# facebookresearch/lightplane

Hardware: AMD Instinct MI355X
Metric: Mrays/sec fwd+bwd, 64^3x16ch triplane @128 samples; peak bwd mem (MB) (higher is better)
Workload: dtype f32

## Files before the change

lightplane_amd/csrc/lp_mfma_common.h:

```cpp
#pragma once
#include <stdlib.h>

#include "lp_device.h"
#include "lp_splat_walk.h"
#include "lp_host.h"
#include "lp_plane_range.h"

namespace lp {

typedef float f32x16 __attribute__((ext_vector_type(16)));

LP_DEV constexpr int featq(int q, int h) { return (q & 3) + 8 * (q >> 2) + 4 * h; }

#define LP_MFMA(a, b, c) __builtin_amdgcn_mfma_f32_32x32x2f32((a), (b), (c), 0, 0, 0)

LP_DEV int opaque_zero() {
  int z = 0;
  asm volatile("" : "+s"(z));
  return z;
}

constexpr int HID = 32;
constexpr int W_LD = 33;
constexpr int WAVES = 4;
// ... 5 lines not shown
constexpr int GM_VOXEL = 2;

struct MfmaParams {
  int64_t w_t1, w_t2, b_t1, b_t2;
  int64_t w_o1, w_o2, b_o1, b_o2;
  int64_t w_c1, w_c2, b_c1, b_c2;
  int ldc2;
  int hid, t2, oh, ch;
  int t1, tg, hin;
  int seg_blocks;
  int seg_fwd;
  uint32_t* relu_dump;
  int tm_rpw;
};

struct Lds {
  static constexpr int WT1 = 0;
  static constexpr int WT2 = WT1 + 32 * W_LD;
  static constexpr int WO1 = WT2 + 32 * W_LD;
  static constexpr int WC1 = WO1 + 32 * W_LD;
  static constexpr int BIAS = WC1 + 32 * W_LD;
  static constexpr int WO2 = BIAS + 4 * 32;
  static constexpr int WC2 = WO2 + 32;
  static constexpr int HB = WC2 + 32 * 4;
  static constexpr int INF = HB + 8;
  static constexpr int FWD_END = INF + MAX_INF;
};

LP_DEV f32x16 load_bias(const float* lds, int which, int h, int zo) {
  const float4* b = reinterpret_cast<const float4*>(lds + Lds::BIAS + which * 32 + 4 * h + zo);
  f32x16 acc;
#pragma unroll
  for (int j = 0; j < 4; ++j) {
    const float4 v = b[2 * j];
    acc[4 * j + 0] = v.x; acc[4 * j + 1] = v.y; acc[4 * j + 2] = v.z; acc[4 * j + 3] = v.w;
  }
  return acc;
}

LP_DEV int wave_min_i(int v) {
#pragma unroll
  for (int m = 32; m >= 1; m >>= 1) { const int o = __shfl_xor(v, m); v = o < v ? o : v; }
  return __builtin_amdgcn_readfirstlane(v);
}
struct WaveRanges {
  unsigned lo3, hi3;
  static constexpr unsigned G = 0x20080200u;
  LP_DEV unsigned mask(int s) const {
    s = __builtin_amdgcn_readfirstlane(s);
    const unsigned sss = (unsigned)(s < 511 ? s : 511) * 0x00100401u;
    return ((sss | G) - lo3) & ((hi3 | G) - sss) & G;
  }
  static constexpr unsigned bit(int g) { return 0x200u << (10 * g); }
};
constexpr int RANGE_MAX_S = 511;
LP_DEV WaveRanges wave_ranges_full() { return WaveRanges{0u, 0x1ff7fdffu}; }
template <int GM>
LP_DEV WaveRanges wave_plane_ranges(const LpRendererArgs& a, const Ray& ray, bool valid, bool plain) {
  WaveRanges w = wave_ranges_full();
  if (GM == GM_GENERIC) return w;
  const int S = a.march.num_samples;
  if (!plain || S > RANGE_MAX_S || __ballot(!valid) != 0) return w;
  const LpGrid* g = a.grid.grids;
  const int W = g[0].W, H = g[0].H, D = (GM == GM_TRIPLANE) ? g[1].D : g[0].D;
  const AxisSpans ax = ray_axis_spans(ray.ox, ray.oy, ray.oz, ray.dx, ray.dy, ray.dz, ray.near_t, ray.far_t, S, W, H, D);
#pragma unroll
  for (int p = 0; p < (GM == GM_TRIPLANE ? 3 : 1); ++p) {
    const SampleSpan sp = (GM == GM_TRIPLANE) ? plane_span(ax, p, S) : voxel_span(ax, S);
    const int lo = wave_min_i(sp.lo), hi = -wave_min_i(-sp.hi);
    if (p == 0) w.lo3 = w.hi3 = 0u;
    w.lo3 |= (unsigned)(hi < lo ? 511 : lo) << (10 * p);
    w.hi3 |= (unsigned)(hi < lo ? 0 : hi) << (10 * p);
  }
  if (GM == GM_VOXEL) {
    w.lo3 *= 0x00100401u;
    w.hi3 *= 0x00100401u;
  }
  w.lo3 = (unsigned)__builtin_amdgcn_readfirstlane((int)w.lo3);
  w.hi3 = (unsigned)__builtin_amdgcn_readfirstlane((int)w.hi3);
  return w;
}

template <int C>
LP_DEV void gather_tap(const float* data, int row, float w, int h, float (&x0)[C / 2]) {
  const float4* src = reinterpret_cast<const float4*>(data + (int64_t)(row < 0 ? 0 : row) * C + 4 * h);
#pragma unroll
  for (int j = 0; j < C / 8; ++j) {
    const float4 v = src[2 * j];
    x0[4 * j + 0] = fmaf(w, v.x, x0[4 * j + 0]);
    x0[4 * j + 1] = fmaf(w, v.y, x0[4 * j + 1]);
    x0[4 * j + 2] = fmaf(w, v.z, x0[4 * j + 2]);
    x0[4 * j + 3] = fmaf(w, v.w, x0[4 * j + 3]);
  }
}

template <int C>
LP_DEV void gather_taps4(const float* data, const int* row, const float* w, float keep, int h, float (&x0)[C / 2]) {
  float4 v[4][C / 8];
#pragma unroll
  for (int k = 0; k < 4; ++k) {
    const float4* src = reinterpret_cast<const float4*>(data + (int64_t)(row[k] < 0 ? 0 : row[k]) * C + 4 * h);
#pragma unroll
    for (int j = 0; j < C / 8; ++j) v[k][j] = src[2 * j];
  }
  __builtin_amdgcn_sched_barrier(0);
#pragma unroll
  for (int k = 0; k < 4; ++k) {
    const float wk = w[k] * keep;
#pragma unroll
    for (int j = 0; j < C / 8; ++j) {
      x0[4 * j + 0] = fmaf(wk, v[k][j].x, x0[4 * j + 0]);
      x0[4 * j + 1] = fmaf(wk, v[k][j].y, x0[4 * j + 1]);
      x0[4 * j + 2] = fmaf(wk, v[k][j].z, x0[4 * j + 2]);
      x0[4 * j + 3] = fmaf(wk, v[k][j].w, x0[4 * j + 3]);
    }
  }
}

template <int C, bool FENCED>
LP_DEV void gather_list(const LpGridList& gl, bool mask_oob, const Ray& ray, float x, float y, float z, int h,
                        float (&x0)[C / 2]) {
#pragma unroll
  for (int q = 0; q < C / 2; ++q) x0[q] = 0.0f;
  const float keep = (mask_oob && !point_in_bounds(x, y, z)) ? 0.0f : 1.0f;
  for (int g = 0; g < gl.n_grids; ++g) {
// ... 486 lines not shown
```

lightplane_amd/csrc/lp_plane_range.h:

```cpp
#pragma once
#include <math.h>

#if defined(__HIPCC__)
#define LP_HD __host__ __device__ inline
#else
#define LP_HD inline
#endif

namespace lp {

struct SampleSpan {
  int lo, hi;
};

LP_HD SampleSpan span_full(int S) { return SampleSpan{0, S - 1}; }
LP_HD SampleSpan span_none(int S) { return SampleSpan{S, -1}; }
LP_HD SampleSpan span_meet(SampleSpan a, SampleSpan b, int S) {
  const SampleSpan m{a.lo > b.lo ? a.lo : b.lo, a.hi < b.hi ? a.hi : b.hi};
  return m.lo > m.hi ? span_none(S) : m;
}
LP_HD SampleSpan span_hull(SampleSpan a, SampleSpan b) {
  return SampleSpan{a.lo < b.lo ? a.lo : b.lo, a.hi > b.hi ? a.hi : b.hi};
}

LP_HD SampleSpan axis_sample_span(float o, float d, float near_t, float far_t, int S, int size) {
  if (S < 2) return span_full(S);
  const float L = 1.0f + 1.0f / (float)size;
  const float per = (float)(S - 1) / (far_t - near_t);
  const float inv = 1.0f / d;
  float s0 = ((-L - o) * inv - near_t) * per;
  float s1 = ((L - o) * inv - near_t) * per;
  if (s0 > s1) { const float t = s0; s0 = s1; s1 = t; }
  const float err = 1.9073486e-6f * fabsf(per) * ((L + fabsf(o)) * fabsf(inv) + fabsf(near_t) + fabsf(far_t));
  if (!(err < 0.5f)) return span_full(S);
  if (!(s0 <= (float)S && s1 >= -1.0f)) return span_none(S);
  const int lo = (int)floorf(fmaxf(s0, 0.0f)) - 1;
  const int hi = (int)ceilf(fminf(s1, (float)(S - 1))) + 1;
  return SampleSpan{lo < 0 ? 0 : lo, hi > S - 1 ? S - 1 : hi};
}

struct AxisSpans {
  SampleSpan x, y, z;
};
LP_HD AxisSpans ray_axis_spans(float ox, float oy, float oz, float dx, float dy, float dz, float near_t, float far_t, int S, int W,
                               int H, int D) {
  return AxisSpans{axis_sample_span(ox, dx, near_t, far_t, S, W), axis_sample_span(oy, dy, near_t, far_t, S, H),
                   axis_sample_span(oz, dz, near_t, far_t, S, D)};
}
LP_HD SampleSpan plane_span(const AxisSpans& a, int g, int S) {
  return g == 0 ? span_meet(a.x, a.y, S) : (g == 1 ? span_meet(a.x, a.z, S) : span_meet(a.y, a.z, S));
}
LP_HD SampleSpan voxel_span(const AxisSpans& a, int S) { return span_meet(span_meet(a.x, a.y, S), a.z, S); }

}
```

lightplane_amd/csrc/lp_renderer_mfma.hip:

```cpp
#include "lp_mfma_common.h"
#include "lp_bf3.h"

namespace lp {

template <int C, int GM, int OCC, int NC, bool SEGF = false>
__global__ void __launch_bounds__(256, OCC) renderer_fwd_bf3(const LpRendererArgs a, const MfmaParams mp) {
  extern __shared__ __attribute__((aligned(16))) float lds[];
  stage_weights_bf3<C>(a, mp, lds, false, 256);
  __syncthreads();
  const float* sm = lds - Lds::BIAS;
  const char* fimg = reinterpret_cast<const char*>(lds) + LdsBf3<C>::FWD_IMG;
  const int lane = threadIdx.x & 63, wave = threadIdx.x >> 6;
  const int h = lane >> 5, r = lane & 31;
  const int seg_len = LP_SEG_LEN * mp.seg_blocks;
  const int n_seg = SEGF ? (a.march.num_samples + seg_len - 1) / seg_len : 1;
  const int blk = SEGF ? (int)blockIdx.x / n_seg : (int)blockIdx.x;
  const int seg = SEGF ? (int)blockIdx.x - blk * n_seg : 0;
  const int64_t ray_id = ((int64_t)blk * WAVES + wave) * RAYS_PER_WAVE + r;
  const bool valid = ray_id < a.rays.n_rays;
  const int64_t rid = valid ? ray_id : 0;
  const Ray ray = load_ray(a.rays, rid);
  float cb[16];
  {
    float enc[16];
    load_encoding(a, rid, h, enc);
    color_prebias_bf3<C>(sm, fimg, lane, enc, cb);
  }
  const int s_tot = a.march.num_samples + a.march.num_samples_inf;
  const int n_ckpt = ckpt_count(a.march);
  const float delta0 = (a.march.num_samples > 1) ? (ray.far_t - ray.near_t) / (float)(a.march.num_samples - 1) : 1.0f;
  float nlt = 0.0f, nlt_lo = 0.0f, t_prev = 1.0f, len = 0.0f, depth_prev = 0.0f;
  int s_last = s_tot - 1;
  float facc[4] = {0.0f, 0.0f, 0.0f, 0.0f};
  Sample<C> nx;
  Act<C> t;
  const int s_lo = SEGF ? seg * seg_len : 0;
  const int s_hi = SEGF ? ((s_lo + seg_len < s_tot) ? s_lo + seg_len : s_tot) : s_tot;
  const bool plain_march = !SEGF && a.march.num_samples_inf == 0 && !a.march.contract_coords && !a.scaffold && !(a.noise_sigma > 0.0f);
  const WaveRanges rg = wave_plane_ranges<GM>(a, ray, valid, plain_march);
  if (SEGF && s_lo > 0) {
    sample_geometry<C>(a, sm, ray, s_lo - 1, nx);
    depth_prev = nx.depth;
  }
  for (int s = s_lo; s < s_hi; ++s) {
    fetch_sample<C, GM, true>(a, sm, ray, s, h, nx, rg.mask(s));
    const float depth = nx.depth, occ = nx.occ;
#pragma unroll
    for (int q = 0; q < C / 2; ++q) t.x0[q] = nx.x0[q];
    const int zo = opaque_zero();
    const Heads hd = decode_bf3<C, NC>(sm, fimg, lane, cb, t, zo);
    const float delta = (s == 0) ? delta0 : depth - depth_prev;
    depth_prev = depth;
    float raw = hd.raw_o;
    if (a.noise_sigma > 0.0f) raw = raw + sample_noise(rid, s, a.rays.n_rays, s_tot, a.noise_seed) * a.noise_sigma;
    const float opacity = a.gain * softplus_f(raw) * occ;
    nlt_add(nlt, nlt_lo, opacity * delta);
    if (!SEGF && a.neg_log_t_ckpt && valid && h == 0) {
      const int ck = ckpt_index(s, a.march);
      if (ck >= 0) *reinterpret_cast<float2*>(a.neg_log_t_ckpt + (ray_id * n_ckpt + ck) * 2) = make_float2(nlt, nlt_lo);
    }
    const float tr = __expf(-nlt);
    const float w = t_prev - tr;
    t_prev = tr;
    len = fmaf(w, depth, len);
#pragma unroll
    for (int c = 0; c < NC; ++c) facc[c] = fmaf(w, sigmoid_f(hd.raw_c[c]) * occ, facc[c]);
    if (a.seg_prefix && valid && h == 0 && (((s + 1) % LP_SEG_LEN) == 0 || s == a.march.num_samples - 1)) {
      float4* dst = reinterpret_cast<float4*>(a.seg_prefix + (ray_id * segment_count(a.march) + s / LP_SEG_LEN) * 8);
      dst[0] = make_float4(len, facc[0], facc[1], facc[2]);
      dst[1] = make_float4(NC == 4 ? facc[3] : 0.0f, nlt, nlt_lo, 0.0f);
    }
    if (a.stop_neg_log_t > 0.0f && __ballot(valid && nlt < a.stop_neg_log_t) == 0) {
      s_last = s;
      break;
    }
  }
  if (!SEGF && valid && h == 0) {
    write_ray_outputs(a, ray_id, len, nlt, facc);
    if (a.neg_log_t_ckpt)
      *reinterpret_cast<float2*>(a.neg_log_t_ckpt + (ray_id * n_ckpt + n_ckpt - 1) * 2) = make_float2((float)s_last, nlt_lo);
  }
}

__global__ void __launch_bounds__(256) renderer_fwd_combine(const LpRendererArgs a, int seg_blocks) {
  const int64_t ray_id = (int64_t)blockIdx.x * 256 + threadIdx.x;
  if (ray_id >= a.rays.n_rays) return;
  const int S = a.march.num_samples;
  const int n_rec = segment_count(a.march), n_ckpt = ckpt_count(a.march);
  float4* rec = reinterpret_cast<float4*>(a.seg_prefix + ray_id * n_rec * 8);
  float n0 = 0.0f, n0_lo = 0.0f, l0 = 0.0f, f0[4] = {0.0f, 0.0f, 0.0f, 0.0f}, t0 = 1.0f;
  float nlt = 0.0f, nlt_lo = 0.0f, len = 0.0f, f[4] = {0.0f, 0.0f, 0.0f, 0.0f};
  for (int b = 0; b < n_rec; ++b) {
    if (b > 0 && b % seg_blocks == 0) {
      n0 = nlt; n0_lo = nlt_lo; l0 = len; t0 = __expf(-nlt);
      for (int c = 0; c < 4; ++c) f0[c] = f[c];
    }
    const float4 r0 = rec[2 * b], r1 = rec[2 * b + 1];
    nlt = n0; nlt_lo = n0_lo;
    nlt_add(nlt, nlt_lo, r1.y);
    nlt_add(nlt, nlt_lo, r1.z);
    len = fmaf(t0, r0.x, l0);
    f[0] = fmaf(t0, r0.y, f0[0]);
    f[1] = fmaf(t0, r0.z, f0[1]);
// ... 188 lines not shown
  return GM_GENERIC;
}

template <typename K>
static int set_lds(K kernel, size_t bytes) {
  const hipError_t e = hipFuncSetAttribute((const void*)kernel, hipFuncAttributeMaxDynamicSharedMemorySize, (int)bytes);
  if (e != hipSuccess) return set_error((int)e, "hipFuncSetAttribute: %s", hipGetErrorString(e));
  return LP_OK;
}

static unsigned n_blocks(const LpRendererArgs& a) {
  return (unsigned)((a.rays.n_rays + WAVES * RAYS_PER_WAVE - 1) / (WAVES * RAYS_PER_WAVE));
}

template <int C, int GM>
static int launch_fwd(const LpRendererArgs& a, const MfmaParams& mp, hipStream_t stream) {
  int rc;
  const bool nc3 = a.color_chn <= 3;
  if (renderer_tm_eligible(a)) {
    MfmaParams mt = mp;
    mt.tm_rpw = renderer_tm_rays_per_wave(a, 768);
    const size_t lds3 = (size_t)LdsBf3<C>::FWD_END;
    const unsigned nb = (unsigned)((a.rays.n_rays + WAVES * mt.tm_rpw - 1) / (WAVES * mt.tm_rpw));
    if (nc3) {
      if ((rc = set_lds(renderer_fwd_bf3_tm<C, GM, 3>, lds3))) return rc;
      hipLaunchKernelGGL((renderer_fwd_bf3_tm<C, GM, 3>), dim3(nb), dim3(256), lds3, stream, a, mt);
    } else {
      if ((rc = set_lds(renderer_fwd_bf3_tm<C, GM, 4>, lds3))) return rc;
      hipLaunchKernelGGL((renderer_fwd_bf3_tm<C, GM, 4>), dim3(nb), dim3(256), lds3, stream, a, mt);
    }
    return LP_OK;
  }
  static const int bf3_occ = getenv("LP_BF3_OCC") ? atoi(getenv("LP_BF3_OCC")) : 0;
  {
    const size_t lds3 = (size_t)LdsBf3<C>::FWD_END;
    const int occ = bf3_occ ? bf3_occ : (a.rays.n_rays > 2 * 32768 ? 3 : 2);
    static const bool seg_fwd = getenv("LP_SEG_FWD") == nullptr || atoi(getenv("LP_SEG_FWD")) != 0;
    if (a.seg_prefix && seg_fwd && !a.seg_forward_off) {
      MfmaParams ms = mp;
      const int n_rec = (a.march.num_samples + LP_SEG_LEN - 1) / LP_SEG_LEN;
      const int m = seg_blocks_for(n_blocks(a), n_rec, 512u);
      ms.seg_blocks = m;
      const unsigned nb = n_blocks(a) * (unsigned)((n_rec + m - 1) / m);
      if (nc3) {
        if ((rc = set_lds(renderer_fwd_bf3<C, GM, 2, 3, true>, lds3))) return rc;
        hipLaunchKernelGGL((renderer_fwd_bf3<C, GM, 2, 3, true>), dim3(nb), dim3(256), lds3, stream, a, ms);
      } else {
        if ((rc = set_lds(renderer_fwd_bf3<C, GM, 2, 4, true>, lds3))) return rc;
        hipLaunchKernelGGL((renderer_fwd_bf3<C, GM, 2, 4, true>), dim3(nb), dim3(256), lds3, stream, a, ms);
      }
      hipLaunchKernelGGL(renderer_fwd_combine, dim3((unsigned)((a.rays.n_rays + 255) / 256)), dim3(256), 0, stream, a, m);
      return LP_OK;
    }
#define LP_BF3_LAUNCH(OCCV, NCV)                                                                                  \
    do {                                                                                                          \
      if ((rc = set_lds(renderer_fwd_bf3<C, GM, OCCV, NCV>, lds3))) return rc;                                   \
      hipLaunchKernelGGL((renderer_fwd_bf3<C, GM, OCCV, NCV>), dim3(n_blocks(a)), dim3(256), lds3, stream, a, mp); \
    } while (0)
    if (occ >= 3) { if (nc3) LP_BF3_LAUNCH(3, 3); else LP_BF3_LAUNCH(3, 4); }
    else { if (nc3) LP_BF3_LAUNCH(2, 3); else LP_BF3_LAUNCH(2, 4); }
#undef LP_BF3_LAUNCH
    return LP_OK;
  }
}

#define LP_DISPATCH_GM(CALL, CV)                                   \
  switch (gm) {                                                    \
    case GM_TRIPLANE: rc = CALL(CV, GM_TRIPLANE); break;           \
    case GM_VOXEL: rc = CALL(CV, GM_VOXEL); break;                 \
    default: rc = CALL(CV, GM_GENERIC); break;                     \
  }

int renderer_forward_mfma(const LpRendererArgs& a, hipStream_t stream) {
  const MfmaParams mp = make_params(a);
  if (n_blocks(a) == 0) return LP_OK;
  const int gm = grid_mode(a);
  int rc;
#define LP_FWD(CV, GMV) launch_fwd<CV, GMV>(a, mp, stream)
  if (a.grid.channels == 16) { LP_DISPATCH_GM(LP_FWD, 16) } else { LP_DISPATCH_GM(LP_FWD, 32) }
#undef LP_FWD
  if (rc) return rc;
  return check_launch("renderer_fwd_mfma");
}

int renderer_backward_mfma(const LpRendererArgs& a, hipStream_t stream) {
  const MfmaParams mp = make_params(a);
  if (n_blocks(a) == 0) return LP_OK;
  return renderer_backward_mfma2(a, mp, grid_mode(a), stream);
}

}
```

lightplane_amd/csrc/lp_renderer_mfma_bwd.h:

```cpp
#pragma once
#include "lp_mfma_common.h"
#include <type_traits>

#include "lp_bf3.h"

namespace lp {

#ifdef LP_ASM_MARKS
#define LP_MARK(n) asm volatile("; LPMARK " n)
#else
#define LP_MARK(n)
#endif
typedef float f32x4 __attribute__((ext_vector_type(4)));
#define LP_MFMA16(a, b, c) __builtin_amdgcn_mfma_f32_16x16x4f32((a), (b), (c), 0, 0, 0)

constexpr int T_LD = 36;

LP_DEV constexpr int pi16(int m) { return m < 4 ? 2 * m : (m < 12 ? 2 * (m - 4) + 1 : 2 * (m - 8)); }

LP_DEV void lds_barrier() { asm volatile("s_waitcnt lgkmcnt(0)\n\ts_barrier" ::: "memory"); }

LP_DEV void tile_store_fm(float* tile, int r, int h, const float (&v)[16]) {
#pragma unroll
  for (int q = 0; q < 16; ++q) tile[featq(q, h) * T_LD + r] = v[q];
// ... 14 lines not shown
    acc = LP_MFMA16(a0.w, b0.w, acc);
    acc = LP_MFMA16(a1.x, b1.x, acc);
    acc = LP_MFMA16(a1.y, b1.y, acc);
    acc = LP_MFMA16(a1.z, b1.z, acc);
    acc = LP_MFMA16(a1.w, b1.w, acc);
    s += ((b0.x + b0.y) + (b0.z + b0.w)) + ((b1.x + b1.y) + (b1.z + b1.w));
  }
  db += s;
  return acc;
}

typedef __bf16 bf16x8_dw __attribute__((ext_vector_type(8)));
#define LP_MFMA16B(a, b, c) \
  __builtin_amdgcn_mfma_f32_16x16x32_bf16(__builtin_bit_cast(bf16x8_dw, (a)), __builtin_bit_cast(bf16x8_dw, (b)), (c), 0, 0, 0)
constexpr int LT_LIMB = rm_bytes(32);

LP_DEV u32x4_t limb_tile_operand(const char* p) {
  typedef __attribute__((address_space(3))) s16x4_t* lds_ptr;
  const s16x4_t a = __builtin_amdgcn_ds_read_tr16_b64_v4i16((lds_ptr)(p));
  const s16x4_t b = __builtin_amdgcn_ds_read_tr16_b64_v4i16((lds_ptr)(p + (rm_off(4, 0) - rm_off(0, 0))));
  const u32x2_t ua = __builtin_bit_cast(u32x2_t, a), ub = __builtin_bit_cast(u32x2_t, b);
  return (u32x4_t){ua.x, ua.y, ub.x, ub.y};
}
template <int STRIDE_BYTES>
LP_DEV f32x4 dw_quadrant_bf(const char* wave0b, int x_off, int y_off, int v0, int v1, f32x4 acc, f32x4& acc_db, unsigned onehot, bool do_db = true) {
  const u32x4_t oh = {onehot, onehot, onehot, onehot};
#pragma unroll 1
  for (int v = v0; v < v1; ++v) {
    const char* base = wave0b + v * STRIDE_BYTES;
    const u32x4_t b2 = limb_tile_operand(base + y_off + LT_LIMB);
    const u32x4_t a1 = limb_tile_operand(base + x_off);
    if (do_db) acc_db = LP_MFMA16B(oh, b2, acc_db);
    acc = LP_MFMA16B(a1, b2, acc);
    const u32x4_t b1 = limb_tile_operand(base + y_off);
    if (do_db) acc_db = LP_MFMA16B(oh, b1, acc_db);
    acc = LP_MFMA16B(a1, b1, acc);
    const u32x4_t a2 = limb_tile_operand(base + x_off + LT_LIMB);
    acc = LP_MFMA16B(a2, b1, acc);
  }
  return acc;
}

struct LdsB3 {
  static constexpr int XT = 0;
  static constexpr int YT = 32 * T_LD;
  static constexpr int TS = 2 * 32 * T_LD;
  static constexpr int PER_WAVE = TS + 5 * 32;
};
template <int C, int NW>
struct Bf3Lds {
  static constexpr int IMG_END = (NW == 8) ? LdsBf3<C>::BWD_END : LdsBf3Rm<C>::END;
  static constexpr int CB = IMG_END + NW * LdsB3::PER_WAVE * 4;
  static constexpr bool CB_LDS = (NW == 8) ? (C == 16) : (CB + NW * 64 * 16 * 4) * 2 <= 160 * 1024;
  static constexpr int TOTAL = CB + (CB_LDS ? NW * 64 * 16 * 4 : 0);
};

template <int C, int GM, bool PLAIN, int NC, int NW, bool SEG = false, bool DUMP = false, bool F32 = false>
__global__ void __launch_bounds__(64 * NW, NW == 8 ? 1 : 2) renderer_bwd_bf3(const LpRendererArgs a, const MfmaParams mp) {
  constexpr int DXL = F32 ? 3 : 2;
  constexpr bool DWB = !F32;
  using M = Lds;
  using L = LdsBf3<C>;
  using R = LdsBf3Rm<C>;
  using B = LdsB3;
  constexpr int WAVES3 = NW;
  extern __shared__ __attribute__((aligned(16))) float lds[];
  if (NW == 8) stage_weights_bf3<C>(a, mp, lds, true, 64 * NW);
  else stage_weights_rm<C>(a, mp, lds, 64 * NW);
  const float* const sm = lds - M::BIAS;
  const char* const fimg = reinterpret_cast<const char*>(lds) + L::FWD_IMG;
  const char* const bimg = reinterpret_cast<const char*>(lds) + L::BWD_IMG;
  const char* const rimg = reinterpret_cast<const char*>(lds);
  const int lane = threadIdx.x & 63;
  const int wave = __builtin_amdgcn_readfirstlane((int)(threadIdx.x >> 6));
  const int h = lane >> 5, r = lane & 31;
  float* const wave0 = reinterpret_cast<float*>(reinterpret_cast<char*>(lds) + Bf3Lds<C, NW>::IMG_END);
  float* const wv = wave0 + wave * B::PER_WAVE;
  float* const xt = wv + B::XT;
  float* const yt = wv + B::YT;
  float* const ts = wv + B::TS;

  constexpr bool seg_on = SEG;
  const int n_rec = seg_on ? segment_count(a.march) : 1;
  const int seg_len = LP_SEG_LEN * mp.seg_blocks;
  const int n_seg = seg_on ? (a.march.num_samples + seg_len - 1) / seg_len : 1;
  const int blk = seg_on ? (int)blockIdx.x / n_seg : (int)blockIdx.x;
  const int seg = seg_on ? (int)blockIdx.x - blk * n_seg : 0;
  const int64_t ray_id = ((int64_t)blk * WAVES3 + wave) * RAYS_PER_WAVE + r;
  const bool valid = ray_id < a.rays.n_rays;
  const int64_t rid = valid ? ray_id : 0;
  const Ray ray = load_ray(a.rays, rid);
  const int s_tot = a.march.num_samples + a.march.num_samples_inf;
  const int n_ckpt = ckpt_count(a.march);
  int s_last_w = s_tot - 1;
  float nlt_lo = 0.0f;
  if (a.neg_log_t_ckpt) {
    const float2 e2 = *reinterpret_cast<const float2*>(a.neg_log_t_ckpt + (rid * n_ckpt + n_ckpt - 1) * 2);
    s_last_w = __builtin_amdgcn_readfirstlane((int)e2.x);
    s_last_w = s_last_w < 0 ? 0 : (s_last_w > s_tot - 1 ? s_tot - 1 : s_last_w);
    nlt_lo = e2.y;
  }
  int s_begin = s_tot - 1;
  if (PLAIN) {
    __syncthreads();
  } else {
    if (lane == 0) ts[0] = (float)s_last_w;
    __syncthreads();
// ... 24 lines not shown
  }
  float dsum[16];
#pragma unroll
  for (int q = 0; q < 16; ++q) dsum[q] = 0.0f;
  float gfeat[4];
#pragma unroll
  for (int c = 0; c < 4; ++c)
    gfeat[c] = (valid && a.grad_feature && c < a.color_chn) ? a.grad_feature[rid * a.color_chn + c] : 0.0f;
  const float g_len = (valid && a.grad_ray_length) ? a.grad_ray_length[rid] : 0.0f;
  const float g_nlt = epilogue_grad_nlt(a, rid, valid, a.neg_log_t[rid],
                                        (valid && a.grad_neg_log_t) ? a.grad_neg_log_t[rid] : 0.0f, gfeat, 4);
  const bool want_params = a.grad_mlp_params != nullptr;
  const float delta0 = (a.march.num_samples > 1) ? (ray.far_t - ray.near_t) / (float)(a.march.num_samples - 1) : 1.0f;

  const int mi = (wave & 3) >> 1, ni = wave & 1;
  const int v0 = 4 * (wave >> 2);
  const int m16 = lane & 15, ka = lane >> 4;
  const int a_off = B::XT + (16 * mi + pi16(m16)) * T_LD + 8 * ka;
  const int b_off = B::YT + (16 * ni + pi16(m16)) * T_LD + 8 * ka;
  auto rho = [](int k) { return (k & 0x15) | ((k & 2) << 2) | ((k & 8) >> 2); };
  char* const xrow = reinterpret_cast<char*>(wv) + B::XT * 4 + rm_off(rho(r), 4 * h);
  char* const yrow = xrow + (B::YT - B::XT) * 4;
  const int xq_off = B::XT * 4 + rm_off(rho(8 * ka + (m16 >> 2)), 4 * (m16 & 3)) + 32 * mi;
  const int yq_off = B::YT * 4 + rm_off(rho(8 * ka + (m16 >> 2)), 4 * (m16 & 3)) + 32 * ni;
  f32x4 dq_b = {0, 0, 0, 0};
  auto onehot = [&](int li) -> unsigned { return (lane & 15) == li ? 0x3F803F80u : 0u; };
  const int a_off_t1 = (C == 16) ? B::XT + pi16(m16) * T_LD + 8 * ka : a_off;
  const int t1_v0 = (C == 16) ? 2 * (wave >> 1) : v0, t1_v1 = (C == 16) ? 2 * (wave >> 1) + 2 : v0 + 4;
  f32x4 dq_t1 = {0, 0, 0, 0}, dq_t2 = {0, 0, 0, 0}, dq_o1 = {0, 0, 0, 0}, dq_c1 = {0, 0, 0, 0};
  float db_t1 = 0.0f, db_t2 = 0.0f, db_o1 = 0.0f, db_c1 = 0.0f;
  float dwo2 = 0.0f, dwc2[4] = {0.0f, 0.0f, 0.0f, 0.0f};
  float dbo2 = 0.0f, dbc2[4] = {0.0f, 0.0f, 0.0f, 0.0f};
  const bool gg = a.grad_grid_list[0] != nullptr;

  float nlt = a.neg_log_t[rid];
  float suffix = 0.0f, p_next = 0.0f;
  if (seg_on) {
    const float4* pj = reinterpret_cast<const float4*>(a.seg_prefix + (rid * n_rec + s_begin / LP_SEG_LEN) * 8);
    const float4* pt = reinterpret_cast<const float4*>(a.seg_prefix + (rid * n_rec + n_rec - 1) * 8);
    const float4 j0 = pj[0], j1 = pj[1], t0 = pt[0];
    nlt = j1.y;
    nlt_lo = j1.z;
    if (seg < n_seg - 1) {
      float rest = g_len * (t0.x - j0.x);
      rest = fmaf(gfeat[0], t0.y - j0.y, rest);
      rest = fmaf(gfeat[1], t0.z - j0.z, rest);
      rest = fmaf(gfeat[2], t0.w - j0.w, rest);
      if (NC == 4) rest = fmaf(gfeat[3], pt[1].x - j1.x, rest);
      suffix = -rest;
    }
  }
  const WaveRanges rg = wave_plane_ranges<GM>(a, ray, valid, PLAIN && !SEG);
  Sample<C> nx;
  fetch_sample<C, GM, false, PLAIN>(a, sm, ray, s_begin, h, nx);
  for (int s = s_begin; s >= s_lo; --s) {
    const bool on = PLAIN || s <= s_last_w;
    const unsigned pm = rg.mask(s);
    const bool ggs = gg && pm != 0u;
    const float depth = nx.depth, occ = nx.occ, x = nx.x, y = nx.y, z = nx.z;
    float x0[C / 2];
#pragma unroll
    for (int q = 0; q < C / 2; ++q) x0[q] = nx.x0[q];
    const int zo = opaque_zero();
    const float* ldz = sm + zo;
    auto Af = [&](auto layer) {
      constexpr int l = decltype(layer)::value;
      if constexpr (NW == 8) return ASlots{fimg + zo, l == 0 ? L::CH_T1 : l == 1 ? L::CH_T2 : l == 2 ? L::CH_O1 : L::CH_C1};
      else return AColsFwd{rimg + zo + (l == 0 ? R::L_T1 : l == 1 ? R::L_T2 : l == 2 ? R::L_O1 : R::L_C1), l == 0 ? R::ST_T1 : R::ST_32};
    };
    auto Ab = [&](auto layer) {
      constexpr int l = decltype(layer)::value;
      if constexpr (NW == 8) return ASlots{bimg + zo, l == 0 ? L::CB_T1 : l == 1 ? L::CB_T2 : l == 2 ? L::CB_O1 : L::CB_C1};
      else return ARowsBwd{rimg + zo + (l == 0 ? R::L_T1 : l == 1 ? R::L_T2 : l == 2 ? R::L_O1 : R::L_C1), l == 0 ? R::ST_T1 : R::ST_32,
                           l == 0 ? C - 1 : 31};
    };
    using I0 = std::integral_constant<int, 0>; using I1 = std::integral_constant<int, 1>;
    using I2 = std::integral_constant<int, 2>; using I3 = std::integral_constant<int, 3>;

    LP_MARK("fwd");
    float h1[16];
    float e[16];
    unsigned ho_mask = 0, hc_mask = 0;
    Heads hd;
    {
      f32x16 acc;
      {
        acc = layer_bf3v<C / 16>(Af(I0{}), lane, x0, load_bias(sm, 0, h, zo));
#pragma unroll
        for (int q = 0; q < 16; ++q) h1[q] = relu_f(acc[q]);
      }
      acc = layer_bf3v<2>(Af(I1{}), lane, h1, load_bias(sm, 1, h, zo));
#pragma unroll
      for (int q = 0; q < 16; ++q) {
        e[q] = relu_f(acc[q]);
      }
      float ho[16], hc[16];
      {
        f32x16 acc_o = load_bias(sm, 2, h, zo), acc_c;
        if (CBL) {
#pragma unroll
          for (int i = 0; i < 4; ++i) {
            const float4 v = *reinterpret_cast<const float4*>(cbt + zo + ((i + cb_rot) & 3) * 4);
            acc_c[4 * i] = v.x; acc_c[4 * i + 1] = v.y; acc_c[4 * i + 2] = v.z; acc_c[4 * i + 3] = v.w;
          }
        } else {
#pragma unroll
          for (int q = 0; q < 16; ++q) acc_c[q] = cb[q];
        }
        layer2_bf3v<2>(Af(I2{}), Af(I3{}), lane, e, acc_o, acc_c);
#pragma unroll
        for (int q = 0; q < 16; ++q) {
          ho[q] = relu_f(acc_o[q]);
          hc[q] = relu_f(acc_c[q]);
        }
      }
      hd = heads_forward<NC>(sm, h, ho, hc, zo);
#pragma unroll
      for (int q = 0; q < 16; ++q) {
        ho_mask = mask_bit(ho_mask, ho[q], q);
        hc_mask = mask_bit(hc_mask, hc[q], q);
      }
      if constexpr (DUMP) {
        unsigned m1 = 0, m2 = 0, mo = 0, mc = 0;
#pragma unroll
        for (int q = 0; q < 16; ++q) {
          const unsigned bit = 1u << featq(q, h);
          m1 |= (h1[q] > 0.0f) ? bit : 0u;
          m2 |= (e[q] > 0.0f) ? bit : 0u;
          mo |= ((ho_mask >> q) & 1u) ? bit : 0u;
          mc |= ((hc_mask >> q) & 1u) ? bit : 0u;
        }
        m1 |= __shfl_xor(m1, 32); m2 |= __shfl_xor(m2, 32); mo |= __shfl_xor(mo, 32); mc |= __shfl_xor(mc, 32);
        if (valid && h == 0) {
          uint32_t* d = mp.relu_dump + (rid * s_tot + s) * 5;
          d[0] = m1; d[1] = m2; d[2] = mo; d[3] = mc; d[4] = on ? 1u : 2u;
        }
      }
      LP_SCHED_FENCE();
      if (want_params) {
        tile_store_fm(xt, r, h, ho);
        tile_store_fm(yt, r, h, hc);
      }
      LP_SCHED_FENCE();
    }

    LP_MARK("compositing");
    const float depth_prev =
        PLAIN ? ray.near_t + lin01((s > 0) ? s - 1 : 0, a.march.num_samples) * (ray.far_t - ray.near_t)
              : sample_depth_tab((s > 0) ? s - 1 : 0, a.march, ray.near_t, ray.far_t, sm + M::INF);
    const float delta = (s == 0) ? delta0 : depth - depth_prev;
    float raw = hd.raw_o;
    if (!PLAIN && a.noise_sigma > 0.0f)
      raw = raw + sample_noise(rid, s, a.rays.n_rays, s_tot, a.noise_seed) * a.noise_sigma;
    const float opacity = a.gain * softplus_f(raw) * occ;
    if (on && a.neg_log_t_ckpt) {
      const int ck = PLAIN ? ((((s + 1) % LP_NLT_CKPT) == 0 || s == s_tot - 1) ? s / LP_NLT_CKPT : -1)
                           : ckpt_index(s, a.march);
      if (ck >= 0) {
        const float2 c2 = *reinterpret_cast<const float2*>(a.neg_log_t_ckpt + (rid * n_ckpt + ck) * 2);
        nlt = c2.x;
        nlt_lo = c2.y;
      }
    }
    const float t_i = __expf(-nlt);
    nlt_add(nlt, nlt_lo, on ? -(opacity * delta) : 0.0f);
    if (!(nlt > 0.0f)) { nlt = 0.0f; nlt_lo = 0.0f; }
    const float t_im1 = __expf(-nlt);
    const float w = t_im1 - t_i;
    float sg[4];
    float p_i = g_len * depth;
#pragma unroll
    for (int c = 0; c < 4; ++c) {
      sg[c] = (c < NC) ? sigmoid_f(hd.raw_c[c]) : 0.0f;
      if (c < NC) p_i = fmaf(gfeat[c], sg[c] * occ, p_i);
    }
    suffix = on ? fmaf(t_i, p_i - p_next, suffix) : suffix;
    p_next = on ? p_i : p_next;
    const float d_a = suffix + g_nlt;
    const bool contrib = valid && on;
    const float dro = contrib ? d_a * delta * a.gain * occ * d_softplus_f(raw) : 0.0f;
    float drc[4];
#pragma unroll
    for (int c = 0; c < 4; ++c) drc[c] = (c < NC && contrib) ? w * gfeat[c] * occ * sg[c] * (1.0f - sg[c]) : 0.0f;

    LP_MARK("heads_bwd");
    float dhc[16];
    {
      const float* wc2 = sm + M::WC2 + 16 * h + opaque_zero();
#pragma unroll
      for (int j = 0; j < 4; ++j) {
#pragma unroll
        for (int i = 0; i < 4; ++i) {
          const int q = 4 * j + i;
          const float4 wc = *reinterpret_cast<const float4*>(wc2 + (8 * j + i) * 4);
          float v = drc[0] * wc.x;
          v = fmaf(drc[1], wc.y, v);
          v = fmaf(drc[2], wc.z, v);
          if (NC > 3) v = fmaf(drc[3], wc.w, v);
          dhc[q] = mask_apply(hc_mask, q, v);
        }
        LP_SCHED_FENCE();
      }
    }
    if (h == 0) {
      dbo2 += dro;
#pragma unroll
      for (int c = 0; c < NC; ++c) dbc2[c] += drc[c];
    }
    if (want_params) {
      if (h == 0) {
        ts[r] = dro;
#pragma unroll
        for (int c = 0; c < NC; ++c) ts[(1 + c) * 32 + r] = drc[c];
      }
      const float* xf = xt + r * T_LD + 16 * h;
      const float* yf = yt + r * T_LD + 16 * h;
      const float* tf = ts + 16 * h;
#pragma unroll
      for (int i = 0; i < 4; ++i) {
        const float4 hov = *reinterpret_cast<const float4*>(xf + 4 * i);
        const float4 hcv = *reinterpret_cast<const float4*>(yf + 4 * i);
        const float4 d0 = *reinterpret_cast<const float4*>(tf + 4 * i);
        dwo2 = fmaf(hov.x, d0.x, dwo2); dwo2 = fmaf(hov.y, d0.y, dwo2);
        dwo2 = fmaf(hov.z, d0.z, dwo2); dwo2 = fmaf(hov.w, d0.w, dwo2);
#pragma unroll
        for (int c = 0; c < NC; ++c) {
          const float4 dc = *reinterpret_cast<const float4*>(tf + (1 + c) * 32 + 4 * i);
          dwc2[c] = fmaf(hcv.x, dc.x, dwc2[c]); dwc2[c] = fmaf(hcv.y, dc.y, dwc2[c]);
          dwc2[c] = fmaf(hcv.z, dc.z, dwc2[c]); dwc2[c] = fmaf(hcv.w, dc.w, dwc2[c]);
        }
        LP_SCHED_FENCE();
      }
    }
    LP_SCHED_FENCE();

    LP_MARK("c1");
// ... 57 lines not shown
        if (want_params) limb_tile_store<2>(xrow, h1);
        acc = layer_dxv<2, DXL>(Ab(I1{}), lane, de, (f32x16){0}, want_params ? yrow : nullptr);
      } else {
        if (want_params) {
          tile_store_fm(xt, r, h, h1);
          tile_store_fm(yt, r, h, de);
        }
        acc = layer_dxv<2, DXL>(Ab(I1{}), lane, de, (f32x16){0});
      }
      if (want_params) {
        lds_barrier();
        if constexpr (DWB) dq_t2 = dw_quadrant_bf<B::PER_WAVE * 4>(reinterpret_cast<const char*>(wave0), xq_off, yq_off, v0, v0 + 4, dq_t2, dq_b, onehot(2));
        else dq_t2 = dw_quadrant<B::PER_WAVE>(wave0, a_off, b_off, v0, v0 + 4, dq_t2, db_t2);
      }
#pragma unroll
      for (int q = 0; q < 16; ++q) dh1[q] = (h1[q] > 0.0f) ? acc[q] : 0.0f;
      if (want_params) lds_barrier();
    }
    LP_SCHED_FENCE();
    LP_MARK("t1");
    {
      if constexpr (DWB) {
        if (want_params) limb_tile_store<C / 16>(xrow, x0);
        if (ggs) {
          acc = layer_dxv<2, DXL>(Ab(I0{}), lane, dh1, (f32x16){0}, want_params ? yrow : nullptr);
        } else if (want_params) {
          limb_tile_store<2>(yrow, dh1);
        }
      } else {
        if (want_params) {
#pragma unroll
          for (int q = 0; q < C / 2; ++q) xt[featq(q, h) * T_LD + r] = x0[q];
          tile_store_fm(yt, r, h, dh1);
        }
        if (ggs) {
          acc = layer_dxv<2, DXL>(Ab(I0{}), lane, dh1, (f32x16){0});
        }
      }
      if (want_params) {
        lds_barrier();
        if constexpr (DWB) dq_t1 = dw_quadrant_bf<B::PER_WAVE * 4>(reinterpret_cast<const char*>(wave0), (C == 16) ? xq_off - 32 * mi : xq_off, yq_off, t1_v0, t1_v1, dq_t1, dq_b, onehot(3));
        else dq_t1 = dw_quadrant<B::PER_WAVE>(wave0, a_off_t1, b_off, t1_v0, t1_v1, dq_t1, db_t1);
        lds_barrier();
      }
    }
    if (ggs) {
#pragma unroll
      for (int q = 0; q < C / 2; ++q) xt[featq(q, h) * DX_LD + r] = acc[q];
    }
    LP_SCHED_FENCE();
    LP_MARK("fetch");
    __builtin_amdgcn_s_setprio(0);
    const bool live = valid && on && !(a.march.mask_out_of_bounds && !point_in_bounds(x, y, z));
    if (s > s_lo) fetch_sample<C, GM, true, PLAIN>(a, sm, ray, s - 1, h, nx, rg.mask(s - 1));
    LP_SCHED_FENCE();
    LP_MARK("scatter");
    if (ggs) {
      if constexpr (GM == GM_TRIPLANE) {
        scatter_triplane<C>(a.grad_grid_list, a.grid, ray.b, x, y, z, live, lane, xt, yt, pm);
      } else {
        const int ng = (GM == GM_VOXEL) ? 1 : a.grid.n_grids;
#pragma unroll 1
        for (int g = 0; g < ng; ++g)
          scatter_grid<C, GM>(a.grad_grid_list[g], a.grid.grids[g], ray.b, x, y, z, live, lane, xt, yt);
      }
    }
  }

  LP_MARK("epilogue");
  {
    f32x16 acc;
    if constexpr (NW == 8) acc = layer_bf3v<2>(ASlots{bimg, L::CB_C1}, lane, dsum, (f32x16){0});
    else acc = layer_bf3v<2>(ARowsBwd{rimg + R::L_C1, R::ST_32, 31}, lane, dsum, (f32x16){0});
    if (valid && a.grad_encoding && !seg_on) {
      float4* dst = reinterpret_cast<float4*>(a.grad_encoding + ray_id * HID + 4 * h);
#pragma unroll
      for (int j = 0; j < 4; ++j) dst[2 * j] = make_float4(acc[4 * j], acc[4 * j + 1], acc[4 * j + 2], acc[4 * j + 3]);
    } else if (valid && a.grad_encoding) {
      float* dst = a.grad_encoding + ray_id * HID + 4 * h;
#pragma unroll
      for (int j = 0; j < 4; ++j)
#pragma unroll
        for (int i = 0; i < 4; ++i) atomic_add_f32(dst + 8 * j + i, acc[4 * j + i]);
    }
  }
  if (want_params) {
    {
      float enc[16];
      load_encoding(a, rid, h, enc);
      if (!valid) {
#pragma unroll
        for (int q = 0; q < 16; ++q) enc[q] = 0.0f;
      }
      __syncthreads();
      if constexpr (DWB) {
        limb_tile_store<2>(xrow, enc);
        limb_tile_store<2>(yrow, dsum);
        lds_barrier();
        dq_c1 = dw_quadrant_bf<B::PER_WAVE * 4>(reinterpret_cast<const char*>(wave0), xq_off, yq_off, v0, v0 + 4, dq_c1, dq_b, 0u, false);
      } else {
        tile_store_fm(xt, r, h, enc);
        tile_store_fm(yt, r, h, dsum);
        float db_unused = 0.0f;
        lds_barrier();
        dq_c1 = dw_quadrant<B::PER_WAVE>(wave0, a_off, b_off, v0, v0 + 4, dq_c1, db_unused);
      }
    }
// ... 114 lines not shown
```

Measured before the change: 31.22.

## Skip MLP work for off-grid samples using a cached zero-feature decode

Samples a wave (or block in backward) never reaches on any plane have all-zero features. For those, the MLP decode is run once per ray and the head outputs are reused. In the forward pass the decoded heads sit in extra LDS. In the backward pass, head and tail off-grid samples are marched with a scalar-only loop that accumulates head gradients, which are then pushed once through a single MLP backward step. This removes per-sample MFMA decode and backward work outside the grid, at the cost of more LDS, an extra block barrier, and more complex control flow.

```diff
diff --git a/lightplane_amd/csrc/lp_mfma_common.h b/lightplane_amd/csrc/lp_mfma_common.h
--- a/lightplane_amd/csrc/lp_mfma_common.h
+++ b/lightplane_amd/csrc/lp_mfma_common.h
@@ -81,6 +81,10 @@
     return ((sss | G) - lo3) & ((hi3 | G) - sss) & G;
   }
   static constexpr unsigned bit(int g) { return 0x200u << (10 * g); }
+  LP_DEV SampleSpan reached() const {
+    const SampleSpan r = packed_reached_span(lo3, hi3);
+    return SampleSpan{__builtin_amdgcn_readfirstlane(r.lo), __builtin_amdgcn_readfirstlane(r.hi)};
+  }
 };
 constexpr int RANGE_MAX_S = 511;
 LP_DEV WaveRanges wave_ranges_full() { return WaveRanges{0u, 0x1ff7fdffu}; }
@@ -98,8 +102,8 @@
     const SampleSpan sp = (GM == GM_TRIPLANE) ? plane_span(ax, p, S) : voxel_span(ax, S);
     const int lo = wave_min_i(sp.lo), hi = -wave_min_i(-sp.hi);
     if (p == 0) w.lo3 = w.hi3 = 0u;
-    w.lo3 |= (unsigned)(hi < lo ? 511 : lo) << (10 * p);
-    w.hi3 |= (unsigned)(hi < lo ? 0 : hi) << (10 * p);
+    w.lo3 |= pack_span_lo(SampleSpan{lo, hi}) << (10 * p);
+    w.hi3 |= pack_span_hi(SampleSpan{lo, hi}) << (10 * p);
   }
   if (GM == GM_VOXEL) {
     w.lo3 *= 0x00100401u;
diff --git a/lightplane_amd/csrc/lp_plane_range.h b/lightplane_amd/csrc/lp_plane_range.h
--- a/lightplane_amd/csrc/lp_plane_range.h
+++ b/lightplane_amd/csrc/lp_plane_range.h
@@ -52,4 +52,26 @@
 }
 LP_HD SampleSpan voxel_span(const AxisSpans& a, int S) { return span_meet(span_meet(a.x, a.y, S), a.z, S); }
 
+constexpr int SPAN_FIELD_MAX = 511;
+LP_HD unsigned pack_span_lo(SampleSpan hull) { return (unsigned)(hull.hi < hull.lo ? SPAN_FIELD_MAX : hull.lo); }
+LP_HD unsigned pack_span_hi(SampleSpan hull) { return (unsigned)(hull.hi < hull.lo ? 0 : hull.hi); }
+LP_HD SampleSpan packed_reached_span(unsigned lo3, unsigned hi3) {
+  SampleSpan r{SPAN_FIELD_MAX, 0};
+  for (int g = 0; g < 3; ++g) {
+    const int lo = (int)((lo3 >> (10 * g)) & 0x1ffu), hi = (int)((hi3 >> (10 * g)) & 0x1ffu);
+    r.lo = lo < r.lo ? lo : r.lo;
+    r.hi = hi > r.hi ? hi : r.hi;
+  }
+  return r;
 }
+struct MarchSplit {
+  int head, tail;
+};
+LP_HD MarchSplit march_split(SampleSpan reached, int S) {
+  if (reached.lo > reached.hi) return MarchSplit{0, 0};
+  const int lo = reached.lo < 0 ? 0 : reached.lo;
+  const int hi = (reached.hi >= SPAN_FIELD_MAX || reached.hi > S - 1) ? S - 1 : reached.hi;
+  return lo > hi ? MarchSplit{0, 0} : MarchSplit{lo, hi + 1};
+}
+
+}
diff --git a/lightplane_amd/csrc/lp_renderer_mfma.hip b/lightplane_amd/csrc/lp_renderer_mfma.hip
--- a/lightplane_amd/csrc/lp_renderer_mfma.hip
+++ b/lightplane_amd/csrc/lp_renderer_mfma.hip
@@ -42,13 +42,36 @@
     sample_geometry<C>(a, sm, ray, s_lo - 1, nx);
     depth_prev = nx.depth;
   }
+  constexpr bool OFFGRID = !SEGF && GM != GM_GENERIC;
+  MarchSplit ms{s_lo, s_hi};
+  float4* const hd0s = reinterpret_cast<float4*>(reinterpret_cast<char*>(lds) + LdsBf3<C>::FWD_END) + 2 * threadIdx.x;
+  if (OFFGRID) {
+    ms = march_split(rg.reached(), s_hi);
+    if (ms.head > 0 || ms.tail < s_hi) {
+#pragma unroll
+      for (int q = 0; q < C / 2; ++q) t.x0[q] = 0.0f;
+      const Heads hd0 = decode_bf3<C, NC>(sm, fimg, lane, cb, t, opaque_zero());
+      hd0s[0] = make_float4(hd0.raw_o, hd0.raw_c[0], hd0.raw_c[1], hd0.raw_c[2]);
+      if (NC == 4) hd0s[1] = make_float4(hd0.raw_c[3], 0.0f, 0.0f, 0.0f);
+    }
+  }
   for (int s = s_lo; s < s_hi; ++s) {
-    fetch_sample<C, GM, true>(a, sm, ray, s, h, nx, rg.mask(s));
+    const bool off = OFFGRID && (s < ms.head || s >= ms.tail);
+    Heads hd;
+    if (off) {
+      sample_geometry<C>(a, sm, ray, s, nx);
+      const float4* src = hd0s + 2 * opaque_zero();
+      const float4 v = src[0];
+      hd.raw_o = v.x; hd.raw_c[0] = v.y; hd.raw_c[1] = v.z; hd.raw_c[2] = v.w;
+      hd.raw_c[3] = (NC == 4) ? src[1].x : 0.0f;
+    } else {
+      fetch_sample<C, GM, true>(a, sm, ray, s, h, nx, rg.mask(s));
+#pragma unroll
+      for (int q = 0; q < C / 2; ++q) t.x0[q] = nx.x0[q];
+      const int zo = opaque_zero();
+      hd = decode_bf3<C, NC>(sm, fimg, lane, cb, t, zo);
+    }
     const float depth = nx.depth, occ = nx.occ;
-#pragma unroll
-    for (int q = 0; q < C / 2; ++q) t.x0[q] = nx.x0[q];
-    const int zo = opaque_zero();
-    const Heads hd = decode_bf3<C, NC>(sm, fimg, lane, cb, t, zo);
     const float delta = (s == 0) ? delta0 : depth - depth_prev;
     depth_prev = depth;
     float raw = hd.raw_o;
@@ -343,10 +366,11 @@
       hipLaunchKernelGGL(renderer_fwd_combine, dim3((unsigned)((a.rays.n_rays + 255) / 256)), dim3(256), 0, stream, a, m);
       return LP_OK;
     }
-#define LP_BF3_LAUNCH(OCCV, NCV)                                                                                  \
-    do {                                                                                                          \
-      if ((rc = set_lds(renderer_fwd_bf3<C, GM, OCCV, NCV>, lds3))) return rc;                                   \
-      hipLaunchKernelGGL((renderer_fwd_bf3<C, GM, OCCV, NCV>), dim3(n_blocks(a)), dim3(256), lds3, stream, a, mp); \
+    const size_t lds_og = lds3 + 256 * 2 * sizeof(float4);
+#define LP_BF3_LAUNCH(OCCV, NCV)                                                                                    \
+    do {                                                                                                            \
+      if ((rc = set_lds(renderer_fwd_bf3<C, GM, OCCV, NCV>, lds_og))) return rc;                                   \
+      hipLaunchKernelGGL((renderer_fwd_bf3<C, GM, OCCV, NCV>), dim3(n_blocks(a)), dim3(256), lds_og, stream, a, mp); \
     } while (0)
     if (occ >= 3) { if (nc3) LP_BF3_LAUNCH(3, 3); else LP_BF3_LAUNCH(3, 4); }
     else { if (nc3) LP_BF3_LAUNCH(2, 3); else LP_BF3_LAUNCH(2, 4); }
diff --git a/lightplane_amd/csrc/lp_renderer_mfma_bwd.h b/lightplane_amd/csrc/lp_renderer_mfma_bwd.h
--- a/lightplane_amd/csrc/lp_renderer_mfma_bwd.h
+++ b/lightplane_amd/csrc/lp_renderer_mfma_bwd.h
@@ -90,7 +90,8 @@
   static constexpr int IMG_END = (NW == 8) ? LdsBf3<C>::BWD_END : LdsBf3Rm<C>::END;
   static constexpr int CB = IMG_END + NW * LdsB3::PER_WAVE * 4;
   static constexpr bool CB_LDS = (NW == 8) ? (C == 16) : (CB + NW * 64 * 16 * 4) * 2 <= 160 * 1024;
-  static constexpr int TOTAL = CB + (CB_LDS ? NW * 64 * 16 * 4 : 0);
+  static constexpr int SPAN = CB + (CB_LDS ? NW * 64 * 16 * 4 : 0);
+  static constexpr int TOTAL = SPAN + NW * 8;
 };
 
 template <int C, int GM, bool PLAIN, int NC, int NW, bool SEG = false, bool DUMP = false, bool F32 = false>
@@ -221,10 +222,150 @@
   }
   const WaveRanges rg = wave_plane_ranges<GM>(a, ray, valid, PLAIN && !SEG);
   Sample<C> nx;
-  fetch_sample<C, GM, false, PLAIN>(a, sm, ray, s_begin, h, nx);
-  for (int s = s_begin; s >= s_lo; --s) {
+
+  constexpr bool OG = PLAIN && !SEG && GM != GM_GENERIC;
+  MarchSplit ms{s_lo, s_begin + 1};
+  bool og_any = false;
+  volatile float og_stash[OG ? 10 : 1];
+  volatile unsigned og_words[(OG && DUMP) ? 4 : 1];
+  auto og_run = [&](int s_from, int s_to) {
+    Heads hd0;
+    hd0.raw_o = og_stash[0];
+#pragma unroll
+    for (int c = 0; c < 4; ++c) hd0.raw_c[c] = (c < NC) ? og_stash[1 + c] : 0.0f;
+    float og_dro = og_stash[5], og_drc[4];
+#pragma unroll
+    for (int c = 0; c < 4; ++c) og_drc[c] = (c < NC) ? og_stash[6 + c] : 0.0f;
+    unsigned words[4] = {0u, 0u, 0u, 0u};
+    if constexpr (DUMP) {
+#pragma unroll
+      for (int k = 0; k < 4; ++k) words[k] = og_words[k];
+    }
+    const float raw = hd0.raw_o;
+    const float opacity = a.gain * softplus_f(raw) * 1.0f;
+    float sg[4];
+#pragma unroll
+    for (int c = 0; c < 4; ++c) sg[c] = (c < NC) ? sigmoid_f(hd0.raw_c[c]) : 0.0f;
+#pragma unroll 1
+    for (int s = s_from; s >= s_to; --s) {
+      const float depth = ray.near_t + lin01(s, a.march.num_samples) * (ray.far_t - ray.near_t);
+      const float depth_prev = ray.near_t + lin01((s > 0) ? s - 1 : 0, a.march.num_samples) * (ray.far_t - ray.near_t);
+      const float delta = (s == 0) ? delta0 : depth - depth_prev;
+      if (a.neg_log_t_ckpt) {
+        const int ck = (((s + 1) % LP_NLT_CKPT) == 0 || s == s_tot - 1) ? s / LP_NLT_CKPT : -1;
+        if (ck >= 0) {
+          const float2 c2 = *reinterpret_cast<const float2*>(a.neg_log_t_ckpt + (rid * n_ckpt + ck) * 2);
+          nlt = c2.x;
+          nlt_lo = c2.y;
+        }
+      }
+      const float t_i = __expf(-nlt);
+      nlt_add(nlt, nlt_lo, -(opacity * delta));
+      if (!(nlt > 0.0f)) { nlt = 0.0f; nlt_lo = 0.0f; }
+      const float t_im1 = __expf(-nlt);
+      const float w = t_im1 - t_i;
+      float p_i = g_len * depth;
+#pragma unroll
+      for (int c = 0; c < NC; ++c) p_i = fmaf(gfeat[c], sg[c] * 1.0f, p_i);
+      suffix = fmaf(t_i, p_i - p_next, suffix);
+      p_next = p_i;
+      const float d_a = suffix + g_nlt;
+      og_dro += valid ? d_a * delta * a.gain * 1.0f * d_softplus_f(raw) : 0.0f;
+#pragma unroll
+      for (int c = 0; c < NC; ++c) og_drc[c] += valid ? w * gfeat[c] * 1.0f * sg[c] * (1.0f - sg[c]) : 0.0f;
+      if constexpr (DUMP) {
+        if (valid && h == 0) {
+          uint32_t* d = mp.relu_dump + (rid * s_tot + s) * 5;
+          d[0] = words[0]; d[1] = words[1]; d[2] = words[2]; d[3] = words[3]; d[4] = 1u;
+        }
+      }
+    }
+    og_stash[5] = og_dro;
+#pragma unroll
+    for (int c = 0; c < NC; ++c) og_stash[6 + c] = og_drc[c];
+  };
+  if constexpr (OG) {
+    int* const spans = reinterpret_cast<int*>(reinterpret_cast<char*>(lds) + Bf3Lds<C, NW>::SPAN);
+    const SampleSpan mine = rg.reached();
+    if (lane == 0) {
+      spans[2 * wave] = mine.lo;
+      spans[2 * wave + 1] = mine.hi;
+    }
+    __syncthreads();
+    SampleSpan hull = mine;
+#pragma unroll
+    for (int v = 0; v < WAVES3; ++v) hull = span_hull(hull, SampleSpan{spans[2 * v], spans[2 * v + 1]});
+    ms = march_split(SampleSpan{__builtin_amdgcn_readfirstlane(hull.lo), __builtin_amdgcn_readfirstlane(hull.hi)}, s_tot);
+    og_any = true;
+    {
+      const int zo = opaque_zero();
+      auto Af0 = [&](int l) { return AColsFwd{rimg + zo + (l == 0 ? R::L_T1 : l == 1 ? R::L_T2 : l == 2 ? R::L_O1 : R::L_C1), l == 0 ? R::ST_T1 : R::ST_32}; };
+      auto As0 = [&](int l) { return ASlots{fimg + zo, l == 0 ? L::CH_T1 : l == 1 ? L::CH_T2 : l == 2 ? L::CH_O1 : L::CH_C1}; };
+      (void)Af0; (void)As0;
+      float z0[C / 2], h1[16], e[16], ho[16], hc[16];
+#pragma unroll
+      for (int q = 0; q < C / 2; ++q) z0[q] = 0.0f;
+      f32x16 acc;
+      if constexpr (NW == 8) acc = layer_bf3v<C / 16>(As0(0), lane, z0, load_bias(sm, 0, h, zo));
+      else acc = layer_bf3v<C / 16>(Af0(0), lane, z0, load_bias(sm, 0, h, zo));
+#pragma unroll
+      for (int q = 0; q < 16; ++q) h1[q] = relu_f(acc[q]);
+      if constexpr (NW == 8) acc = layer_bf3v<2>(As0(1), lane, h1, load_bias(sm, 1, h, zo));
+      else acc = layer_bf3v<2>(Af0(1), lane, h1, load_bias(sm, 1, h, zo));
+#pragma unroll
+      for (int q = 0; q < 16; ++q) e[q] = relu_f(acc[q]);
+      f32x16 acc_o = load_bias(sm, 2, h, zo), acc_c;
+      if (CBL) {
+#pragma unroll
+        for (int i = 0; i < 4; ++i) {
+          const float4 v = *reinterpret_cast<const float4*>(cbt + zo + ((i + cb_rot) & 3) * 4);
+          acc_c[4 * i] = v.x; acc_c[4 * i + 1] = v.y; acc_c[4 * i + 2] = v.z; acc_c[4 * i + 3] = v.w;
+        }
+      } else {
+#pragma unroll
+        for (int q = 0; q < 16; ++q) acc_c[q] = cb[q];
+      }
+      if constexpr (NW == 8) layer2_bf3v<2>(As0(2), As0(3), lane, e, acc_o, acc_c);
+      else layer2_bf3v<2>(Af0(2), Af0(3), lane, e, acc_o, acc_c);
+#pragma unroll
+      for (int q = 0; q < 16; ++q) {
+        ho[q] = relu_f(acc_o[q]);
+        hc[q] = relu_f(acc_c[q]);
+      }
+      const Heads hd0 = heads_forward<NC>(sm, h, ho, hc, zo);
+      og_stash[0] = hd0.raw_o;
+#pragma unroll
+      for (int c = 0; c < NC; ++c) og_stash[1 + c] = hd0.raw_c[c];
+      og_stash[5] = 0.0f;
+#pragma unroll
+      for (int c = 0; c < NC; ++c) og_stash[6 + c] = 0.0f;
+      if constexpr (DUMP) {
+        unsigned words[4] = {0u, 0u, 0u, 0u};
+#pragma unroll
+        for (int q = 0; q < 16; ++q) {
+          const unsigned bit = 1u << featq(q, h);
+          words[0] |= (h1[q] > 0.0f) ? bit : 0u;
+          words[1] |= (e[q] > 0.0f) ? bit : 0u;
+          words[2] |= (ho[q] > 0.0f) ? bit : 0u;
+          words[3] |= (hc[q] > 0.0f) ? bit : 0u;
+        }
+#pragma unroll
+        for (int k = 0; k < 4; ++k) og_words[k] = words[k] | __shfl_xor(words[k], 32);
+      }
+      og_run(s_begin, ms.tail);
+    }
+  }
+  fetch_sample<C, GM, false, PLAIN>(a, sm, ray, ms.tail > 0 ? ms.tail - 1 : 0, h, nx);
+  const int s_end = ms.head - (og_any ? 1 : 0);
+  for (int s = ms.tail - 1; s >= s_end; --s) {
+    const bool fl = OG && s == s_end;
+    if (OG && __builtin_expect(fl, 0)) {
+      og_run(s_end, 0);
+#pragma unroll
+      for (int q = 0; q < C / 2; ++q) nx.x0[q] = 0.0f;
+    }
     const bool on = PLAIN || s <= s_last_w;
-    const unsigned pm = rg.mask(s);
+    const unsigned pm = fl ? 0u : rg.mask(s);
     const bool ggs = gg && pm != 0u;
     const float depth = nx.depth, occ = nx.occ, x = nx.x, y = nx.y, z = nx.z;
     float x0[C / 2];
@@ -300,7 +441,7 @@
           mc |= ((hc_mask >> q) & 1u) ? bit : 0u;
         }
         m1 |= __shfl_xor(m1, 32); m2 |= __shfl_xor(m2, 32); mo |= __shfl_xor(mo, 32); mc |= __shfl_xor(mc, 32);
-        if (valid && h == 0) {
+        if (valid && h == 0 && !fl) {
           uint32_t* d = mp.relu_dump + (rid * s_tot + s) * 5;
           d[0] = m1; d[1] = m2; d[2] = mo; d[3] = mc; d[4] = on ? 1u : 2u;
         }
@@ -347,10 +488,15 @@
     p_next = on ? p_i : p_next;
     const float d_a = suffix + g_nlt;
     const bool contrib = valid && on;
-    const float dro = contrib ? d_a * delta * a.gain * occ * d_softplus_f(raw) : 0.0f;
+    float dro = contrib ? d_a * delta * a.gain * occ * d_softplus_f(raw) : 0.0f;
     float drc[4];
 #pragma unroll
     for (int c = 0; c < 4; ++c) drc[c] = (c < NC && contrib) ? w * gfeat[c] * occ * sg[c] * (1.0f - sg[c]) : 0.0f;
+    if (OG && fl) {
+      dro = og_stash[5];
+#pragma unroll
+      for (int c = 0; c < NC; ++c) drc[c] = og_stash[6 + c];
+    }
 
     LP_MARK("heads_bwd");
     float dhc[16];
@@ -514,7 +660,7 @@
     LP_MARK("fetch");
     __builtin_amdgcn_s_setprio(0);
     const bool live = valid && on && !(a.march.mask_out_of_bounds && !point_in_bounds(x, y, z));
-    if (s > s_lo) fetch_sample<C, GM, true, PLAIN>(a, sm, ray, s - 1, h, nx, rg.mask(s - 1));
+    if (s > s_end + (OG ? 1 : 0)) fetch_sample<C, GM, true, PLAIN>(a, sm, ray, s - 1, h, nx, rg.mask(s - 1));
     LP_SCHED_FENCE();
     LP_MARK("scatter");
     if (ggs) {
```

New measurement: 31.18. About the same (-0.1%).
